# Rose-STL-Lab/spherical-dyffusion

Hardware: AMD Instinct MI355X
Metric: forecast-steps/sec (180x360, 63ch), 25-member ensemble DYffusion sampling, whole job (higher is better)
Workload: dtype f32 tensors; every GEMM-class kernel (1x1 convs, fused MLP, Legendre analysis/synthesis, dhconv) as 3-pass split-f16 MFMA with f32 accumulation; FFT / norms / pointwise in f32 (statistics f64); 1 GPU; 25-member ensemble x horizon-6 DYffusion sampling pass (6 forecaster + 10 interpolator SFNO forwards, dropout stream on, AR feedback), 180x360, 63 state + 2 forcing channels, embed 256, 8 blocks; horizon=6, relayed_members=0, parallelism=members of one initial condition sharded over GPUs, no data-path collective

## Files before the change

### spherical-dyffusion_amd/csrc/mlp_h3.hip

```cpp
#include <cstdlib>
#include <vector>
#include <cmath>
#include <type_traits>

#include "common.h"

typedef const sdy_f16x8 __attribute__((address_space(1)))* wptr_t;
typedef _Float16 f16x4 __attribute__((ext_vector_type(4)));

namespace {

constexpr int ME = 256;
constexpr int MH = 512;
constexpr int TN = 64;
constexpr int HC = 128;
constexpr int NCH = MH / HC;
constexpr int KS1 = ME / 16;
constexpr int KSC = HC / 16;
constexpr int RING = 16;
constexpr int NGROUPS = NCH * 2 * RING;
static_assert(KS1 == RING && 2 * KSC == RING, "ring slot = index inside a block");
constexpr float SX = SDY_ACT_SX;

struct MlpParams {
  const float* x; long x_bs;
  int x_tiled;
  const float* pa; const float* pd;
  const sdy_f16x8* w;
  const float* b1; const float* b2;
  float* out; long out_bs;
  const float* add; long add_bs;
  const float* add_a; const float* add_d;
  int HW, B;
  float s1, s2;
  uint32_t drop_thr; float drop_scale;
  uint32_t seed_lo, seed_hi, stream1, stream2, call, batch_offset;
  int rows_per_call;
  const float* batch_scale;
  double* stats;
  const float* keep_h; const float* keep_o;
  unsigned* flags;
  unsigned* head;
  unsigned long long* stamps;
  SdyImgMap omap;
  int add_local;
};

__device__ __forceinline__ int px_swz(int px) { return (px & 15) ^ (((px >> 4) & 1) * 3); }
__device__ __forceinline__ int xs_off(int px, int c) { return px * ME + (((c & 16) | ((c ^ px_swz(px)) & 15)) << 3); }
__device__ __forceinline__ int hs_off(int px, int c) { return px * HC + (((c ^ px_swz(px)) & 15) << 3); }

template <bool DROP, bool INJECT = false>
__global__ __launch_bounds__(256, 1) void mlp_h3_kernel(const MlpParams p) {
  extern __shared__ __attribute__((aligned(16))) unsigned char smem[];
  _Float16* Xs_hi = reinterpret_cast<_Float16*>(smem);
  _Float16* Xs_lo = Xs_hi + TN * ME;
  _Float16* Hs = Xs_lo + TN * ME;
  float* Cf = reinterpret_cast<float*>(Hs + 4 * TN * HC);
  float* Cb2 = Cf + 4 * ME;

  const int tid = threadIdx.x, lane = tid & 63;
  const int wave = __builtin_amdgcn_readfirstlane(tid >> 6);
  int h = lane >> 5, l31 = lane & 31;
  const int tpi = (p.HW + TN - 1) / TN;
  const int ntiles = tpi * p.B;
  const int t_per = (ntiles + (int)gridDim.x - 1) / (int)gridDim.x;
  const int t_begin = (int)blockIdx.x * t_per;
  const int t_end = (t_begin + t_per < ntiles) ? t_begin + t_per : ntiles;
  int z = 0, zo = 0, n0 = 0;
  bool full = true;

  sdy_f16x8 r_hi[RING], r_lo[RING];
  auto wbase_of = [&](int ln) { return (wptr_t)(p.w + (size_t)wave * (NGROUPS + RING) * SDY_GROUP + ln); };
  wptr_t wp = wbase_of(lane);
#pragma unroll
  for (int s = 0; s < RING; ++s) {
    r_hi[s] = wp[s * SDY_GROUP];
    r_lo[s] = wp[s * SDY_GROUP + 64];
  }
  wp += RING * SDY_GROUP;

  int q0 = tid & 15, o0 = tid >> 4;
  f32x4 xr[2][8];
  const float* pf_base = nullptr;
  const float* res_base = nullptr;
  unsigned pf_off = 0u;
  int pf_rs = 0;
  auto prefetch_setup = [&](int t) {
    const int zz = t / tpi, nn = (t - zz * tpi) * TN;
    const bool ok = nn + 4 * q0 < p.HW;
    pf_base = p.x + (long)zz * p.x_bs + (p.x_tiled ? (long)(t - zz * tpi) * (ME * TN) : 0L);
    pf_rs = p.x_tiled ? TN : p.HW;
    pf_off = p.x_tiled ? (unsigned)(8 * o0 * TN + 4 * q0) * 4u : (unsigned)(8 * o0 * p.HW + (ok ? nn + 4 * q0 : 0)) * 4u;
  };
  auto prefetch_piece = [&](int piece) {
    const int oc = piece >> 3, e = piece & 7;
    xr[oc][e] = sdy_ld16s(pf_base + (long)(8 * 16 * oc + e) * pf_rs, pf_off);
  };
  auto prefetch_x = [&](int t) {
    const int zz = t / tpi, nn = (t - zz * tpi) * TN;
    const bool ok = nn + 4 * q0 < p.HW;
    const float* xz = p.x + (long)zz * p.x_bs + (p.x_tiled ? (long)(t - zz * tpi) * (ME * TN) : 0L);
    const int rs = p.x_tiled ? TN : p.HW;
    const unsigned xo = p.x_tiled ? (unsigned)(8 * o0 * TN + 4 * q0) * 4u : (unsigned)(8 * o0 * p.HW + (ok ? nn + 4 * q0 : 0)) * 4u;
#pragma unroll
    for (int oc = 0; oc < 2; ++oc)
#pragma unroll
      for (int e = 0; e < 8; ++e) xr[oc][e] = sdy_ld16s(xz + (long)(8 * 16 * oc + e) * rs, xo);
  };
  auto load_coeffs = [&](int zz) {
    const int t = 64 * wave + (int)__builtin_amdgcn_mbcnt_hi(~0u, __builtin_amdgcn_mbcnt_lo(~0u, 0u));
    const long c = (long)zz * ME + t, co = (long)sdy_img(p.omap, zz) * ME + t;
    Cf[t] = p.pa ? p.pa[c] * SX : SX;
    Cf[ME + t] = p.pa ? p.pd[c] * SX : 0.0f;
    Cf[2 * ME + t] = p.add_a ? p.add_a[co] : 1.0f;
    Cf[3 * ME + t] = p.add_a ? p.add_d[co] : 0.0f;
  };
  Cb2[tid] = DROP ? p.b2[tid] * p.drop_scale : p.b2[tid];
  if (t_begin < t_end) load_coeffs(t_begin / tpi);
  __syncthreads();
  if (t_begin < t_end) prefetch_x(t_begin);
  double psum[16], psq[16];
#pragma unroll
  for (int i = 0; i < 16; ++i) { psum[i] = 0.0; psq[i] = 0.0; }

  for (int tile = t_begin; tile < t_end; ++tile) {
  asm volatile("" : "+v"(l31), "+v"(h), "+v"(q0), "+v"(o0));
  const int tile_it = tile - t_begin;
  auto stamp = [&](int i) {
#if SDY_STAMPS_ON
    if (p.stamps && blockIdx.x == 3 && tid == 0 && tile_it >= 2 && tile_it < 6)
      p.stamps[(tile_it - 2) * 16 + i] = __builtin_amdgcn_s_memtime();
#else
    (void)i; (void)tile_it;
    if (p.stamps && tid == 0) asm volatile("s_nop 0");
#endif
  };
  stamp(0);
  z = tile / tpi;
  zo = sdy_img(p.omap, z);
  n0 = (tile - z * tpi) * TN;
  full = n0 + TN <= p.HW;

  auto stage_x = [&](auto full_t) {
    constexpr bool kFull = decltype(full_t)::value;
    float amax = 0.0f;
    const bool ok = kFull || (n0 + 4 * q0 < p.HW);
#pragma unroll
    for (int oc = 0; oc < 2; ++oc) {
      float av[8], dv[8];
      {
        const int c0 = 8 * (o0 + 16 * oc);
        const f32x4 a0 = *reinterpret_cast<const f32x4*>(Cf + c0), a1 = *reinterpret_cast<const f32x4*>(Cf + c0 + 4);
        const f32x4 d0 = *reinterpret_cast<const f32x4*>(Cf + ME + c0), d1 = *reinterpret_cast<const f32x4*>(Cf + ME + c0 + 4);
#pragma unroll
        for (int e = 0; e < 4; ++e) { av[e] = a0[e]; av[e + 4] = a1[e]; dv[e] = d0[e]; dv[e + 4] = d1[e]; }
      }
#pragma unroll
      for (int pp = 0; pp < 4; ++pp) {
        const int px = 4 * q0 + pp;
        sdy_f16x8 vh, vl;
        float v[8];
#pragma unroll
        for (int e = 0; e < 8; ++e) v[e] = (kFull || ok) ? fmaf(xr[oc][e][pp], av[e], dv[e]) : 0.0f;
        sdy_split8(v, vh, vl, amax);
        const int off = xs_off(px, o0 + 16 * oc);
        *reinterpret_cast<sdy_f16x8*>(Xs_hi + off) = vh;
        *reinterpret_cast<sdy_f16x8*>(Xs_lo + off) = vl;
      }
    }
    sdy_flag_range(p.flags, amax, p.head);
  };
  if (full) stage_x(std::true_type{});
  else stage_x(std::false_type{});
  __syncthreads();

  f32x16 oacc[2][2];
  f32x4 rres[16];
  const int e_col = n0 + 4 * (tid & 15);
  const bool e_ok = full || e_col < p.HW;
  const unsigned e_ro = (unsigned)((tid >> 4) * p.HW + (e_ok ? e_col : 0)) * 4u;

  constexpr bool do_drop = DROP;
  const int zq = zo / p.rows_per_call, zt = zo - zq * p.rows_per_call;
  const uint32_t call_z = p.call + (uint32_t)zq;
  const uint32_t c1_base = (uint32_t)(((uint64_t)(zt + p.batch_offset) * (uint64_t)(MH >> 2)) & 0xFFFFFFFFu);

  f32x16 acc[2];
  f32x4 bv[4];
  auto load_bias = [&](int hc) {
    const int row0 = HC * hc + 32 * wave + 4 * h;
#pragma unroll
    for (int g4 = 0; g4 < 4; ++g4) bv[g4] = *reinterpret_cast<const f32x4*>(p.b1 + row0 + 8 * g4);
  };
#ifndef SDY_MLP_PINNED
#define SDY_MLP_PINNED 1
#endif
  static_assert(SDY_MLP_PINNED, "the ahead-of-time Philox rounds ride on the pinned fc1 loop");
  uint32_t mw[4][4];
  uint32_t ac0 = 0, ac1 = 0, ac2 = 0, ac3 = 0, ak0 = 0, ak1 = 0;
  constexpr int PR = SDY_PHILOX_ROUNDS;
  constexpr int PSTEP = 96 / (4 * PR);
  static_assert(PSTEP >= 2, "at most one round behind every other MFMA of fc1");
  auto philox_ahead = [&](int hc, int idx) {
    const int g4 = idx / PR, rnd = idx % PR;
    if (rnd == 0) {
      const int row0 = HC * hc + 32 * wave + 4 * h;
      ac0 = (uint32_t)(n0 + l31); ac1 = c1_base + (uint32_t)((row0 + 8 * g4) >> 2); ac2 = p.stream1; ac3 = call_z;
      ak0 = p.seed_lo; ak1 = p.seed_hi;
    }
    const uint64_t p0 = (uint64_t)0xD2511F53u * ac0, p1 = (uint64_t)0xCD9E8D57u * ac2;
    const uint32_t m0 = (uint32_t)(p1 >> 32) ^ ac1 ^ ak0, m2 = (uint32_t)(p0 >> 32) ^ ac3 ^ ak1;
    ac0 = m0; ac1 = (uint32_t)p1; ac2 = m2; ac3 = (uint32_t)p0;
    ak0 += 0x9E3779B9u; ak1 += 0xBB67AE85u;
    if (rnd == PR - 1) { mw[g4][0] = ac0; mw[g4][1] = ac1; mw[g4][2] = ac2; mw[g4][3] = ac3; }
  };
  auto fc1 = [&](int hc_fc1) {
#pragma unroll
    for (int j = 0; j < 2; ++j)
#pragma unroll
      for (int r = 0; r < 16; ++r) acc[j][r] = 0.0f;
    sdy_f16x8 bh[2][2], bl[2][2];
    auto ldb1 = [&](int set, int ks, int part) {
      const int j = part & 1;
      const int off = xs_off(32 * j + l31, 2 * ks + h);
      if (part < 2) bh[set][j] = *reinterpret_cast<const sdy_f16x8*>(Xs_hi + off);
      else bl[set][j] = *reinterpret_cast<const sdy_f16x8*>(Xs_lo + off);
    };
#pragma unroll
    for (int part = 0; part < 4; ++part) ldb1(0, 0, part);
#pragma unroll
    for (int ks = 0; ks < KS1; ++ks) {
      const int c = ks & 1;
      if constexpr (SDY_MLP_PINNED) {
      __builtin_amdgcn_sched_barrier(0);
      const sdy_f16x8 a_lo = r_lo[ks], a_hi = r_hi[ks];
#pragma unroll
      for (int k = 0; k < 6; ++k) {
        const int j = k & 1;
        if (SDY_H3_PASSES == 3 || k >= 4)
          acc[j] = __builtin_amdgcn_mfma_f32_32x32x16_f16(k < 2 ? a_lo : a_hi, (k >= 2 && k < 4) ? bl[c][j] : bh[c][j], acc[j], 0, 0, 0);
        if (k < 4) { if (ks + 1 < KS1) ldb1(c ^ 1, ks + 1, k); }
        else if (k == 4) r_lo[ks] = wp[ks * SDY_GROUP + 64];
        else r_hi[ks] = wp[ks * SDY_GROUP];
        if (DROP && !INJECT && (6 * ks + k) % PSTEP == 0 && (6 * ks + k) / PSTEP < 4 * PR) philox_ahead(hc_fc1, (6 * ks + k) / PSTEP);
        __builtin_amdgcn_sched_barrier(0);
      }
      } else {
      if (ks + 1 < KS1) {
#pragma unroll
        for (int part = 0; part < 4; ++part) ldb1(c ^ 1, ks + 1, part);
      }
#pragma unroll
      for (int j = 0; j < 2; ++j) SDY_CROSS_TERM(acc[j] = __builtin_amdgcn_mfma_f32_32x32x16_f16(r_lo[ks], bh[c][j], acc[j], 0, 0, 0));
#pragma unroll
      for (int j = 0; j < 2; ++j) SDY_CROSS_TERM(acc[j] = __builtin_amdgcn_mfma_f32_32x32x16_f16(r_hi[ks], bl[c][j], acc[j], 0, 0, 0));
#pragma unroll
      for (int j = 0; j < 2; ++j) acc[j] = __builtin_amdgcn_mfma_f32_32x32x16_f16(r_hi[ks], bh[c][j], acc[j], 0, 0, 0);
      r_hi[ks] = wp[ks * SDY_GROUP];
      r_lo[ks] = wp[ks * SDY_GROUP + 64];
#pragma unroll
      for (int k = 0; k < 4; ++k) {
        __builtin_amdgcn_sched_group_barrier(0x008, 1, 0);
        __builtin_amdgcn_sched_group_barrier(0x100, 1, 0);
      }
#pragma unroll
      for (int k = 0; k < 2; ++k) {
        __builtin_amdgcn_sched_group_barrier(0x008, 1, 0);
        __builtin_amdgcn_sched_group_barrier(0x020, 1, 0);
      }
      __builtin_amdgcn_sched_barrier(0);
      }
    }
    wp += RING * SDY_GROUP;
  };
  struct Piece {
    float v[4], t[4], e[4], q[4];
  };
  auto keep_h_at = [&](int row, int px) {
    const int pix = (n0 + px < p.HW) ? n0 + px : p.HW - 1;
    return p.keep_h[((long)zo * MH + row) * p.HW + pix] != 0.0f;
  };
  auto chain_stage = [&](Piece& s, int st, int hc, int j, int g4) {
    const int row0 = HC * hc + 32 * wave + 4 * h;
    const int px = 32 * j + l31;
    switch (st) {
      case 0: {
        const f32x4 b4 = bv[g4];
#pragma unroll
        for (int r = 0; r < 4; r += 2) {
          const sdy_gf2 v2 = sdy_gf2{acc[j][4 * g4 + r], acc[j][4 * g4 + r + 1]} * p.s1 + sdy_gf2{b4[r], b4[r + 1]};
          s.v[r] = v2.x; s.v[r + 1] = v2.y;
        }
        break;
      }
      case 1:
#pragma unroll
        for (int r = 0; r < 4; r += 2) {
          const sdy_gf2 v2 = {s.v[r], s.v[r + 1]};
          const sdy_gf2 t2 = __builtin_elementwise_abs(v2) * (0.3275911f * 0.70710678118654752440f) + 1.0f;
          const sdy_gf2 e2 = v2 * v2;
          s.t[r] = t2.x; s.t[r + 1] = t2.y;
          s.e[r] = e2.x; s.e[r + 1] = e2.y;
        }
        break;
      case 2: {
        s.t[0] = __builtin_amdgcn_rcpf(s.t[0]); s.t[1] = __builtin_amdgcn_rcpf(s.t[1]);
        const sdy_gf2 e2 = sdy_gf2{s.e[0], s.e[1]} * (-0.5f * 1.44269504088896340736f);
        s.e[0] = e2.x; s.e[1] = e2.y;
        break;
      }
      case 3: {
        s.t[2] = __builtin_amdgcn_rcpf(s.t[2]); s.t[3] = __builtin_amdgcn_rcpf(s.t[3]);
        const sdy_gf2 e2 = sdy_gf2{s.e[2], s.e[3]} * (-0.5f * 1.44269504088896340736f);
        s.e[2] = e2.x; s.e[3] = e2.y;
        break;
      }
      case 4: s.e[0] = __builtin_amdgcn_exp2f(s.e[0]); s.e[1] = __builtin_amdgcn_exp2f(s.e[1]); break;
      case 5: s.e[2] = __builtin_amdgcn_exp2f(s.e[2]); s.e[3] = __builtin_amdgcn_exp2f(s.e[3]); break;
      case 6:
#pragma unroll
        for (int r = 0; r < 4; r += 2) {
          const sdy_gf2 t2 = {s.t[r], s.t[r + 1]};
          sdy_gf2 q2 = t2 * (1.061405429f * (0.5f * SX)) + (-1.453152027f * (0.5f * SX));
          q2 = q2 * t2 + (1.421413741f * (0.5f * SX));
          s.q[r] = q2.x; s.q[r + 1] = q2.y;
        }
        break;
      case 7:
#pragma unroll
        for (int r = 0; r < 4; r += 2) {
          const sdy_gf2 t2 = {s.t[r], s.t[r + 1]};
          sdy_gf2 q2 = sdy_gf2{s.q[r], s.q[r + 1]} * t2 + (-0.284496736f * (0.5f * SX));
          q2 = q2 * t2 + (0.254829592f * (0.5f * SX));
          s.q[r] = q2.x; s.q[r + 1] = q2.y;
        }
        break;
      case 8:
#pragma unroll
        for (int r = 0; r < 4; r += 2) {
          const sdy_gf2 q2 = sdy_gf2{s.q[r], s.q[r + 1]} * sdy_gf2{s.t[r], s.t[r + 1]} * sdy_gf2{s.e[r], s.e[r + 1]};
          s.q[r] = q2.x; s.q[r + 1] = q2.y;
        }
        break;
      case 9:
#pragma unroll
        for (int r = 0; r < 4; r += 2) {
          const sdy_gf2 v2 = {s.v[r], s.v[r + 1]};
          const sdy_gf2 o2 = v2 * (0.5f * SX) + __builtin_elementwise_abs(v2) * ((0.5f * SX) - sdy_gf2{s.q[r], s.q[r + 1]});
          s.v[r] = o2.x; s.v[r + 1] = o2.y;
        }
        break;
      case 10: {
        if (do_drop) {
#pragma unroll
          for (int r = 0; r < 4; ++r) {
            bool keep;
            if constexpr (INJECT) keep = keep_h_at(row0 + 8 * g4 + r, px);
            else keep = sdy_keep16(mw[g4][r], j, p.drop_thr);
            s.v[r] = keep ? s.v[r] : 0.0f;
          }
        }
        break;
      }
      default: {
        _Float16* Hh = Hs + (hc & 1) * (2 * TN * HC);
        _Float16* Hl = Hh + TN * HC;
        f16x4 vh, vl;
#pragma unroll
        for (int r = 0; r < 4; r += 2) {
          const sdy_f32x2 x2 = {s.v[r], s.v[r + 1]};
          const sdy_f16x2 h2 = __builtin_convertvector(x2, sdy_f16x2);
          const sdy_f16x2 l2 = __builtin_convertvector(x2 - __builtin_convertvector(h2, sdy_f32x2), sdy_f16x2);
          vh[r] = h2[0]; vh[r + 1] = h2[1];
          vl[r] = l2[0]; vl[r + 1] = l2[1];
        }
        const int off = hs_off(px, 4 * wave + g4) + 4 * h;
        *reinterpret_cast<f16x4*>(Hh + off) = vh;
        *reinterpret_cast<f16x4*>(Hl + off) = vl;
      }
    }
  };
  auto chain_slot = [&](Piece& s, int st, int hc, int j, int g4) {
    const int row0 = HC * hc + 32 * wave + 4 * h;
    const int px = 32 * j + l31;
    constexpr float CT = 0.3275911f * 0.70710678118654752440f, KAP = -0.5f * 1.44269504088896340736f, HS = 0.5f * SX;
    constexpr float A5 = 1.061405429f * HS, A4 = -1.453152027f * HS, A3 = 1.421413741f * HS, A2 = -0.284496736f * HS,
                    A1 = 0.254829592f * HS;
    switch (st) {
      case 0: {
        const f32x4 b4 = bv[g4];
#pragma unroll
        for (int r = 0; r < 4; ++r) s.v[r] = fmaf(acc[j][4 * g4 + r], p.s1, b4[r]);
        break;
      }
      case 1:
#pragma unroll
        for (int r = 0; r < 4; ++r) s.t[r] = fmaf(__builtin_fabsf(s.v[r]), CT, 1.0f);
        s.e[0] = s.v[0] * KAP; s.e[1] = s.v[1] * KAP;
        break;
      case 2:
        s.t[0] = __builtin_amdgcn_rcpf(s.t[0]); s.t[1] = __builtin_amdgcn_rcpf(s.t[1]);
        s.e[2] = s.v[2] * KAP; s.e[3] = s.v[3] * KAP;
        s.e[0] *= s.v[0]; s.e[1] *= s.v[1];
        break;
      case 3:
        s.t[2] = __builtin_amdgcn_rcpf(s.t[2]); s.t[3] = __builtin_amdgcn_rcpf(s.t[3]);
        s.e[2] *= s.v[2]; s.e[3] *= s.v[3];
        s.q[0] = fmaf(s.t[0], A5, A4); s.q[1] = fmaf(s.t[1], A5, A4);
        break;
      case 4:
        s.e[0] = __builtin_amdgcn_exp2f(s.e[0]); s.e[1] = __builtin_amdgcn_exp2f(s.e[1]);
        s.q[2] = fmaf(s.t[2], A5, A4); s.q[3] = fmaf(s.t[3], A5, A4);
        s.q[0] = fmaf(s.q[0], s.t[0], A3); s.q[1] = fmaf(s.q[1], s.t[1], A3);
        break;
      case 5:
        s.e[2] = __builtin_amdgcn_exp2f(s.e[2]); s.e[3] = __builtin_amdgcn_exp2f(s.e[3]);
        s.q[2] = fmaf(s.q[2], s.t[2], A3); s.q[3] = fmaf(s.q[3], s.t[3], A3);
        s.q[0] = fmaf(s.q[0], s.t[0], A2); s.q[1] = fmaf(s.q[1], s.t[1], A2);
        break;
      case 6:
        s.q[2] = fmaf(s.q[2], s.t[2], A2); s.q[3] = fmaf(s.q[3], s.t[3], A2);
#pragma unroll
        for (int r = 0; r < 4; ++r) s.q[r] = fmaf(s.q[r], s.t[r], A1);
        break;
      case 7:
#pragma unroll
        for (int r = 0; r < 4; ++r) s.q[r] *= s.t[r];
        s.q[0] = fmaf(-s.q[0], s.e[0], HS); s.q[1] = fmaf(-s.q[1], s.e[1], HS);
        break;
      case 8:
        s.q[2] = fmaf(-s.q[2], s.e[2], HS); s.q[3] = fmaf(-s.q[3], s.e[3], HS);
#pragma unroll
        for (int r = 0; r < 4; ++r) s.q[r] *= __builtin_fabsf(s.v[r]);
        break;
      case 9:
#pragma unroll
        for (int r = 0; r < 4; ++r) s.v[r] = fmaf(s.v[r], HS, s.q[r]);
        if (do_drop) {
#pragma unroll
          for (int r = 0; r < 4; ++r) {
            bool keep;
            if constexpr (INJECT) keep = keep_h_at(row0 + 8 * g4 + r, px);
            else keep = sdy_keep16(mw[g4][r], j, p.drop_thr);
            s.v[r] = keep ? s.v[r] : 0.0f;
          }
        }
        break;
      case 10: {
#pragma unroll
        for (int r = 0; r < 4; r += 2) {
          const sdy_f16x2 h2 = __builtin_convertvector(sdy_f32x2{s.v[r], s.v[r + 1]}, sdy_f16x2);
          s.e[r >> 1] = __builtin_bit_cast(float, h2);
          s.t[r] = s.v[r] - (float)h2[0]; s.t[r + 1] = s.v[r + 1] - (float)h2[1];
        }
        break;
      }
      default: {
        _Float16* Hh = Hs + (hc & 1) * (2 * TN * HC);
        _Float16* Hl = Hh + TN * HC;
        f16x4 vh, vl;
#pragma unroll
        for (int r = 0; r < 4; r += 2) {
          const sdy_f16x2 h2 = __builtin_bit_cast(sdy_f16x2, s.e[r >> 1]);
          const sdy_f16x2 l2 = __builtin_convertvector(sdy_f32x2{s.t[r], s.t[r + 1]}, sdy_f16x2);
          vh[r] = h2[0]; vh[r + 1] = h2[1];
          vl[r] = l2[0]; vl[r + 1] = l2[1];
        }
        const int off = hs_off(px, 4 * wave + g4) + 4 * h;
        *reinterpret_cast<f16x4*>(Hh + off) = vh;
        *reinterpret_cast<f16x4*>(Hl + off) = vl;
      }
    }
  };
#ifndef SDY_MLP_SCALAR_CHAIN
#define SDY_MLP_SCALAR_CHAIN 1
#endif
  auto chain_piece = [&](int hc, int j, int g4) {
    Piece s;
#pragma unroll
    for (int st = 0; st < 12; ++st) chain_stage(s, st, hc, j, g4);
  };
  auto fc2 = [&](int hc2, auto with_chain) {
    constexpr bool CHAIN = decltype(with_chain)::value;
    const _Float16* Hh = Hs + (hc2 & 1) * (2 * TN * HC);
    const _Float16* Hl = Hh + TN * HC;
    sdy_f16x8 bh[2][2], bl[2][2];
    auto ldb = [&](int set, int t) {
#pragma unroll
      for (int j = 0; j < 2; ++j) {
        const int off = hs_off(32 * j + l31, 2 * t + h);
        bh[set][j] = *reinterpret_cast<const sdy_f16x8*>(Hh + off);
        bl[set][j] = *reinterpret_cast<const sdy_f16x8*>(Hl + off);
      }
    };
    auto ldb1 = [&](int set, int t, int part) {
      const int j = part & 1;
      const int off = hs_off(32 * j + l31, 2 * t + h);
      if (part < 2) bh[set][j] = *reinterpret_cast<const sdy_f16x8*>(Hh + off);
      else bl[set][j] = *reinterpret_cast<const sdy_f16x8*>(Hl + off);
    };
    ldb(0, 0);
#pragma unroll
    for (int t = 0; t < KSC; ++t) {
      const int c = t & 1;
      if (!SDY_MLP_PINNED && t + 1 < KSC) ldb(c ^ 1, t + 1);
      __builtin_amdgcn_sched_barrier(0);
      Piece ps;
#pragma unroll
      for (int mi = 0; mi < 2; ++mi) {
        const int s = 2 * t + mi;
#pragma unroll
        for (int k = 0; k < 6; ++k) {
          const int j = k & 1;
          const sdy_f16x8 a = (k < 2) ? r_lo[s] : r_hi[s];
          const sdy_f16x8 b = (k >= 2 && k < 4) ? bl[c][j] : bh[c][j];
          if (SDY_H3_PASSES == 3 || k >= 4) oacc[mi][j] = __builtin_amdgcn_mfma_f32_32x32x16_f16(a, b, oacc[mi][j], 0, 0, 0);
          if (SDY_MLP_PINNED && mi == 0 && k < 4 && t + 1 < KSC) ldb1(c ^ 1, t + 1, k);
          if (SDY_MLP_PINNED && !CHAIN) __builtin_amdgcn_sched_barrier(0);
          if constexpr (CHAIN) {
            if (SDY_MLP_SCALAR_CHAIN) chain_slot(ps, 6 * mi + k, hc2 + 1, t & 1, t >> 1);
            else chain_stage(ps, 6 * mi + k, hc2 + 1, t & 1, t >> 1);
            __builtin_amdgcn_sched_barrier(0);
          }
        }
        r_hi[s] = wp[s * SDY_GROUP];
        r_lo[s] = wp[s * SDY_GROUP + 64];
        __builtin_amdgcn_sched_barrier(0);
      }
    }
    wp += RING * SDY_GROUP;
  };
  using T_ = std::integral_constant<bool, true>;
  using F_ = std::integral_constant<bool, false>;

  stamp(1);
  load_bias(0);
  fc1(0);
  stamp(2);
#pragma unroll
  for (int pc = 0; pc < 8; ++pc) chain_piece(0, pc & 1, pc >> 1);
  stamp(3);
  __syncthreads();
  stamp(4);
  load_bias(1);
  fc1(1);
  stamp(5);
#pragma unroll
  for (int mi = 0; mi < 2; ++mi)
#pragma unroll
    for (int j = 0; j < 2; ++j)
#pragma unroll
      for (int r = 0; r < 16; ++r) oacc[mi][j][r] = 0.0f;
#pragma unroll 1
  for (int hc = 1; hc < NCH; ++hc) {
    fc2(hc - 1, T_{});
    stamp(4 + 2 * hc);
    __syncthreads();
    if (hc < NCH - 1) {
      load_bias(hc + 1);
      fc1(hc + 1);
    }
    stamp(5 + 2 * hc);
  }
  {
    int ln = lane;
    asm volatile("" : "+v"(ln));
    wp = wbase_of(ln);
  }
  asm volatile("" : "+v"(wp));
  {
    const int nt = tile + 1;
    prefetch_setup(nt < t_end ? nt : tile);
  }
  fc2(NCH - 1, F_{});
  stamp(12);
  {
    res_base = p.add ? p.add + (long)(p.add_local ? z : zo) * p.add_bs : p.x + (long)z * p.x_bs;
  }

  {
    const float bscale = p.batch_scale ? p.batch_scale[zo] : 1.0f;
    const float s2e = do_drop ? p.s2 * p.drop_scale * p.drop_scale : p.s2;
    const uint32_t c1_base2 = (uint32_t)(((uint64_t)(zt + p.batch_offset) * (uint64_t)(ME >> 2)) & 0xFFFFFFFFu);
    float* Os = reinterpret_cast<float*>(smem);
#pragma unroll
    for (int mi = 0; mi < 2; ++mi) {
      const int row0 = 64 * wave + 32 * mi + 4 * h;
      f32x4 bv[4];
#pragma unroll
      for (int g4 = 0; g4 < 4; ++g4) bv[g4] = *reinterpret_cast<const f32x4*>(Cb2 + row0 + 8 * g4);
#pragma unroll
      for (int g4 = 0; g4 < 4; ++g4) {
        uint32_t words[4] = {0xFFFFFFFFu, 0xFFFFFFFFu, 0xFFFFFFFFu, 0xFFFFFFFFu};
        if (do_drop && !INJECT) {
          const philox4 w = philox4x32((uint32_t)(n0 + l31), c1_base2 + (uint32_t)((row0 + 8 * g4) >> 2), p.stream2,
                                          call_z, p.seed_lo, p.seed_hi);
          words[0] = w.x; words[1] = w.y; words[2] = w.z; words[3] = w.w;
        }
#pragma unroll
        for (int j = 0; j < 2; ++j) {
          const int px = 32 * j + l31;
#pragma unroll
          for (int r4 = 0; r4 < 4; r4 += 2) {
            sdy_gf2 o = sdy_gf2{oacc[mi][j][4 * g4 + r4], oacc[mi][j][4 * g4 + r4 + 1]} * s2e +
                        sdy_gf2{bv[g4][r4], bv[g4][r4 + 1]};
            if (do_drop) {
              if constexpr (INJECT) {
                const int pix = (n0 + px < p.HW) ? n0 + px : p.HW - 1;
                const float* km = p.keep_o + ((long)zo * ME + row0 + 8 * g4 + r4) * p.HW + pix;
                o = sdy_gf2{km[0] != 0.0f ? o.x : 0.0f, km[p.HW] != 0.0f ? o.y : 0.0f};
              } else {
                o = sdy_gf2{sdy_keep16(words[r4], j, p.drop_thr) ? o.x : 0.0f,
                            sdy_keep16(words[r4 + 1], j, p.drop_thr) ? o.y : 0.0f};
              }
            }
            o = o * bscale;
            Os[(row0 + 8 * g4 + r4) * TN + px] = o.x;
            Os[(row0 + 8 * g4 + r4 + 1) * TN + px] = o.y;
          }
        }
        {
          const int i0 = 2 * (4 * mi + g4);
          rres[i0] = sdy_ld16s(res_base + (long)(16 * i0) * p.HW, e_ro);
          rres[i0 + 1] = sdy_ld16s(res_base + (long)(16 * (i0 + 1)) * p.HW, e_ro);
          prefetch_piece(i0);
          prefetch_piece(i0 + 1);
        }
      }
    }
    stamp(13);
    __syncthreads();
    stamp(14);
    if (e_ok) {
      float* oz = p.out + (long)zo * p.out_bs;
      const float* os = Os + (tid >> 4) * TN + 4 * (tid & 15);
#pragma unroll
      for (int i = 0; i < 16; ++i) {
        const int row = (tid >> 4) + 16 * i;
        f32x4 v = *reinterpret_cast<const f32x4*>(os + 16 * i * TN);
        if (p.add) v += rres[i] * Cf[2 * ME + row] + Cf[3 * ME + row];
        sdy_st16s(oz + (long)(16 * i) * p.HW, e_ro, v);
        if (p.stats) {
          psum[i] += (double)sdy_quad_sum(v);
          psq[i] += (double)sdy_quad_sumsq(v);
        }
      }
    }
    if (p.stats) {
      const int nt = tile + 1;
      if (nt >= t_end || nt / tpi != z) {
#pragma unroll
        for (int i = 0; i < 16; ++i) {
          double s1 = psum[i], s2 = psq[i];
#pragma unroll
          for (int m = 1; m < 16; m <<= 1) {
            s1 += __shfl_xor(s1, m, 64);
            s2 += __shfl_xor(s2, m, 64);
          }
          if ((tid & 15) == 0) {
            double* st = p.stats + ((long)zo * ME + (tid >> 4) + 16 * i) * 2;
            __hip_atomic_fetch_add(st, s1, __ATOMIC_RELAXED, __HIP_MEMORY_SCOPE_AGENT);
            __hip_atomic_fetch_add(st + 1, s2, __ATOMIC_RELAXED, __HIP_MEMORY_SCOPE_AGENT);
          }
          psum[i] = 0.0; psq[i] = 0.0;
        }
      }
    }
  }
  stamp(15);
  __syncthreads();
  {
    const int nt = tile + 1;
    if (nt < t_end && nt / tpi != z) {
      load_coeffs(nt / tpi);
      __syncthreads();
    }
  }
  }
}

}

#ifndef SDY_MLP_INJECT_TU
#if SDY_STAMPS_ON
static unsigned long long* g_stamps = nullptr;
SDY_DEBUG_EXPORT int sdy_mlp_h3_debug_stamps(unsigned long long* host64) {
  if (!g_stamps || !host64) return SDY_ERR_STATE;
  SDY_HIP_TRY(hipDeviceSynchronize());
  SDY_HIP_TRY(hipMemcpy(host64, g_stamps, 64 * sizeof(unsigned long long), hipMemcpyDeviceToHost));
  return SDY_OK;
}
#endif

extern "C" int sdy_mlp_h3_supported(int E, int hidden) { return (E == ME && hidden == MH) ? 1 : 0; }

extern "C" size_t sdy_mlp_h3_pack_bytes(int E, int hidden) {
  if (!sdy_mlp_h3_supported(E, hidden)) return 0;
  return (size_t)4 * (NGROUPS + RING) * SDY_GROUP * sizeof(sdy_f16x8);
}

extern "C" int sdy_mlp_h3_pack(const float* w1_host, const float* w2_host, int E, int hidden, void* packed_dev,
                               float* scale1, float* scale2) {
  if (!w1_host || !w2_host || !packed_dev || !scale1 || !scale2) return SDY_ERR_ARG;
  if (!sdy_mlp_h3_supported(E, hidden)) return SDY_ERR_UNSUPPORTED;
  const float s1 = sdy_h3_scale(sdy_h3_absmax(w1_host, (size_t)E * hidden));
  const float s2 = sdy_h3_scale(sdy_h3_absmax(w2_host, (size_t)E * hidden));
  const size_t gh = (size_t)SDY_GROUP * 8;
  std::vector<_Float16> buf((size_t)4 * (NGROUPS + RING) * gh, (_Float16)0.0f);
  for (int w = 0; w < 4; ++w) {
    _Float16* d = buf.data() + (size_t)w * (NGROUPS + RING) * gh;
    auto put_fc1 = [&](int hc) {
      for (int ks = 0; ks < KS1; ++ks, d += gh) {
        const float* blk = w1_host + (size_t)(128 * hc + 32 * w) * ME + 16 * ks;
        sdy_h3_put_group(d, s1, [&](int r, int k) { return blk[(size_t)r * ME + k]; });
      }
    };
    auto put_fc2 = [&](int hc) {
      for (int t = 0; t < KSC; ++t)
        for (int mi = 0; mi < 2; ++mi, d += gh) {
          const float* blk = w2_host + (size_t)(64 * w + 32 * mi) * MH + 16 * (KSC * hc + t);
          sdy_h3_put_group(d, s2, [&](int r, int k) { return blk[(size_t)r * MH + k]; });
        }
    };
    put_fc1(0);
    put_fc1(1);
    for (int hc = 1; hc < NCH; ++hc) {
      put_fc2(hc - 1);
      if (hc < NCH - 1) put_fc1(hc + 1);
    }
    put_fc2(NCH - 1);
  }
  SDY_HIP_TRY(hipMemcpy(packed_dev, buf.data(), buf.size() * sizeof(_Float16), hipMemcpyHostToDevice));
  *scale1 = s1;
  *scale2 = s2;
  return SDY_OK;
}

#endif

int sdy_mlp_h3_inject(const sdy_mlp_args* a, void* stream);

#ifdef SDY_MLP_INJECT_TU
int sdy_mlp_h3_inject(const sdy_mlp_args* a, void* stream) {
#else
extern "C" int sdy_mlp_h3(const sdy_mlp_args* a, void* stream) {
  if (a && (a->keep_hidden || a->keep_out)) {
    if (!a->keep_hidden || !a->keep_out || !(a->drop_p > 0.0f)) return SDY_ERR_ARG;
    return sdy_mlp_h3_inject(a, stream);
  }
#endif
  if (!a || !a->x || !a->w || !a->b1 || !a->b2 || !a->out) return SDY_ERR_ARG;
  if (a->B <= 0 || a->HW <= 0) return SDY_ERR_ARG;
  if (!sdy_mlp_h3_supported(a->E, a->hidden)) return SDY_ERR_UNSUPPORTED;
  if ((a->pa == nullptr) != (a->pd == nullptr) || (a->add_a == nullptr) != (a->add_d == nullptr)) return SDY_ERR_ARG;
  if ((a->HW & 3) || (a->x_bstride & 3) || (a->out_bstride & 3) || (a->add && (a->add_bstride & 3))) return SDY_ERR_ALIGN;
  if ((long)a->HW * ME * 4 >= (1L << 32)) return SDY_ERR_UNSUPPORTED;
  if (a->drop_p < 0.0f || a->drop_p >= 1.0f) return SDY_ERR_ARG;
  if (a->B > 65535) return SDY_ERR_UNSUPPORTED;
  MlpParams p{};
  p.x = a->x; p.x_bs = a->x_bstride; p.x_tiled = a->x_tiled; p.pa = a->pa; p.pd = a->pd;
  if (a->x_tiled && !a->add) return SDY_ERR_ARG;
  p.w = reinterpret_cast<const sdy_f16x8*>(a->w);
  p.b1 = a->b1; p.b2 = a->b2;
  p.out = a->out; p.out_bs = a->out_bstride; p.add = a->add; p.add_bs = a->add_bstride;
  p.add_a = a->add ? a->add_a : nullptr; p.add_d = a->add ? a->add_d : nullptr;
  p.HW = a->HW; p.B = a->B;
  p.s1 = 1.0f / (a->w1_scale * SX);
  p.s2 = 1.0f / (a->w2_scale * SX);
  if (a->drop_p > 0.0f) {
    p.drop_thr = sdy_drop_threshold16(a->drop_p);
    if (p.drop_thr == 0u) p.drop_thr = 1u;
    p.drop_scale = 1.0f / (1.0f - a->drop_p);
  }
  p.seed_lo = (uint32_t)(a->seed & 0xFFFFFFFFu); p.seed_hi = (uint32_t)(a->seed >> 32);
  p.stream1 = a->stream_fc1; p.stream2 = a->stream_fc2; p.call = a->call; p.batch_offset = a->batch_offset;
  if (a->rows_per_call < 0 || (!a->out_rows && a->rows_per_call > 0 && a->B % a->rows_per_call)) return SDY_ERR_ARG;
  if (a->out_rows && a->rows_per_call == 0) return SDY_ERR_ARG;
  p.rows_per_call = a->rows_per_call > 0 ? a->rows_per_call : a->B;
  p.batch_scale = a->batch_scale;
  p.stats = a->stats;
  p.keep_h = a->keep_hidden; p.keep_o = a->keep_out;
  if (a->out_rows && !a->add) return SDY_ERR_ARG;
  if (a->add_by_launch_row && (!a->out_rows || a->add_a)) return SDY_ERR_ARG;
  p.add_local = a->add_by_launch_row ? 1 : 0;
  SDY_TRY(sdy_img_map_fill(p.omap, a->out_rows, a->B));
  SDY_TRY(sdy_flags_ptr(&p.flags));
  SDY_TRY(sdy_headroom_ptr(SDY_RANGE_MLP, &p.head));
  p.stamps = nullptr;
#if SDY_STAMPS_ON && !defined(SDY_MLP_INJECT_TU)
  if (std::getenv("SDY_MLP_STAMPS")) {
    if (!g_stamps) SDY_HIP_TRY(hipMalloc(&g_stamps, 64 * sizeof(unsigned long long)));
    p.stamps = g_stamps;
  }
#endif
  int n_cu = 0;
  SDY_TRY(sdy_cu_count(&n_cu));
  const long ntiles = (long)((a->HW + TN - 1) / TN) * a->B;
  dim3 grid((unsigned)(ntiles < n_cu ? ntiles : n_cu));
  constexpr size_t smem = (size_t)(2 * TN * ME + 4 * TN * HC) * sizeof(_Float16) + 5 * ME * sizeof(float);
  static SdyOncePerDevice once;
  std::atomic<bool>* attr_done = nullptr;
  SDY_TRY(once.slot(&attr_done));
#ifdef SDY_MLP_INJECT_TU
  if (!*attr_done) {
    SDY_HIP_TRY(hipFuncSetAttribute(reinterpret_cast<const void*>(&mlp_h3_kernel<true, true>),
                                    hipFuncAttributeMaxDynamicSharedMemorySize, (int)smem));
    *attr_done = true;
  }
  hipLaunchKernelGGL((mlp_h3_kernel<true, true>), grid, dim3(256), smem, (hipStream_t)stream, p);
#else
  if (!*attr_done) {
    SDY_HIP_TRY(hipFuncSetAttribute(reinterpret_cast<const void*>(&mlp_h3_kernel<false>),
                                    hipFuncAttributeMaxDynamicSharedMemorySize, (int)smem));
    SDY_HIP_TRY(hipFuncSetAttribute(reinterpret_cast<const void*>(&mlp_h3_kernel<true>),
                                    hipFuncAttributeMaxDynamicSharedMemorySize, (int)smem));
    *attr_done = true;
  }
  if (p.drop_thr != 0u)
    hipLaunchKernelGGL(mlp_h3_kernel<true>, grid, dim3(256), smem, (hipStream_t)stream, p);
  else
    hipLaunchKernelGGL(mlp_h3_kernel<false>, grid, dim3(256), smem, (hipStream_t)stream, p);
#endif
  return sdy_launch_status();
}
```

Measured before the change: 163.4 member-forecast-steps/s.

## Stage next tile's x split into swapped LDS region during output epilogue

The shared-memory x image and the hidden double buffer now swap regions each tile. This lets the f16 hi/lo split of the next tile's input be written to the free region while the current tile's output rows are stored. The aim is to remove the serial staging phase and its barrier at the top of each tile by overlapping it with epilogue global stores. In exchange, coefficient loading is split into x and add halves, with an extra sync when the image changes, and correctness now depends on careful region aliasing.

Result: no change. 163.6 member-forecast-steps/s, median of 6 (+0.1%).

```diff
diff --git a/spherical-dyffusion_amd/csrc/mlp_h3.hip b/spherical-dyffusion_amd/csrc/mlp_h3.hip
--- a/spherical-dyffusion_amd/csrc/mlp_h3.hip
+++ b/spherical-dyffusion_amd/csrc/mlp_h3.hip
@@ -21,6 +21,20 @@
 constexpr int NGROUPS = NCH * 2 * RING;
 static_assert(KS1 == RING && 2 * KSC == RING, "ring slot = index inside a block");
 constexpr float SX = SDY_ACT_SX;
+constexpr unsigned REGION = 2 * TN * ME * sizeof(_Float16);
+static_assert(REGION == 4 * TN * HC * sizeof(_Float16), "the x image and the hidden double buffer exchange storage");
+#ifdef SDY_MLP_NO_REGION_SWAP
+constexpr bool SWAP = false;
+#else
+constexpr bool SWAP = true;
+#endif
+#ifndef SDY_MLP_SPLIT0_AT
+#define SDY_MLP_SPLIT0_AT 16
+#endif
+#ifndef SDY_MLP_SPLIT1_AT
+#define SDY_MLP_SPLIT1_AT 16
+#endif
+static_assert(0 <= SDY_MLP_SPLIT0_AT && SDY_MLP_SPLIT0_AT <= SDY_MLP_SPLIT1_AT && SDY_MLP_SPLIT1_AT <= 16, "store rounds");
 
 struct MlpParams {
   const float* x; long x_bs;
@@ -53,10 +67,8 @@
 template <bool DROP, bool INJECT = false>
 __global__ __launch_bounds__(256, 1) void mlp_h3_kernel(const MlpParams p) {
   extern __shared__ __attribute__((aligned(16))) unsigned char smem[];
-  _Float16* Xs_hi = reinterpret_cast<_Float16*>(smem);
-  _Float16* Xs_lo = Xs_hi + TN * ME;
-  _Float16* Hs = Xs_lo + TN * ME;
-  float* Cf = reinterpret_cast<float*>(Hs + 4 * TN * HC);
+  unsigned xreg = 0u;
+  float* Cf = reinterpret_cast<float*>(smem + 2 * REGION);
   float* Cb2 = Cf + 4 * ME;
 
   const int tid = threadIdx.x, lane = tid & 63;
@@ -108,21 +120,68 @@
 #pragma unroll
       for (int e = 0; e < 8; ++e) xr[oc][e] = sdy_ld16s(xz + (long)(8 * 16 * oc + e) * rs, xo);
   };
-  auto load_coeffs = [&](int zz) {
+  auto load_coeffs = [&](int zz, bool x_half, bool add_half) {
     const int t = 64 * wave + (int)__builtin_amdgcn_mbcnt_hi(~0u, __builtin_amdgcn_mbcnt_lo(~0u, 0u));
     const long c = (long)zz * ME + t, co = (long)sdy_img(p.omap, zz) * ME + t;
-    Cf[t] = p.pa ? p.pa[c] * SX : SX;
-    Cf[ME + t] = p.pa ? p.pd[c] * SX : 0.0f;
-    Cf[2 * ME + t] = p.add_a ? p.add_a[co] : 1.0f;
-    Cf[3 * ME + t] = p.add_a ? p.add_d[co] : 0.0f;
+    if (x_half) {
+      Cf[t] = p.pa ? p.pa[c] * SX : SX;
+      Cf[ME + t] = p.pa ? p.pd[c] * SX : 0.0f;
+    }
+    if (add_half) {
+      Cf[2 * ME + t] = p.add_a ? p.add_a[co] : 1.0f;
+      Cf[3 * ME + t] = p.add_a ? p.add_d[co] : 0.0f;
+    }
+  };
+  auto stage_half = [&](auto full_t, int oc, _Float16* Xh, _Float16* Xl, int nn, float& amax) {
+    constexpr bool kFull = decltype(full_t)::value;
+    const bool ok = kFull || (nn + 4 * q0 < p.HW);
+    float av[8], dv[8];
+    {
+      const int c0 = 8 * (o0 + 16 * oc);
+      const f32x4 a0 = *reinterpret_cast<const f32x4*>(Cf + c0), a1 = *reinterpret_cast<const f32x4*>(Cf + c0 + 4);
+      const f32x4 d0 = *reinterpret_cast<const f32x4*>(Cf + ME + c0), d1 = *reinterpret_cast<const f32x4*>(Cf + ME + c0 + 4);
+#pragma unroll
+      for (int e = 0; e < 4; ++e) { av[e] = a0[e]; av[e + 4] = a1[e]; dv[e] = d0[e]; dv[e + 4] = d1[e]; }
+    }
+#pragma unroll
+    for (int pp = 0; pp < 4; ++pp) {
+      const int px = 4 * q0 + pp;
+      sdy_f16x8 vh, vl;
+      float v[8];
+#pragma unroll
+      for (int e = 0; e < 8; ++e) v[e] = (kFull || ok) ? fmaf(xr[oc][e][pp], av[e], dv[e]) : 0.0f;
+      sdy_split8(v, vh, vl, amax);
+      const int off = xs_off(px, o0 + 16 * oc);
+      *reinterpret_cast<sdy_f16x8*>(Xh + off) = vh;
+      *reinterpret_cast<sdy_f16x8*>(Xl + off) = vl;
+    }
+  };
+  auto stage_x = [&](bool full_tile, _Float16* Xh, _Float16* Xl, int nn) {
+    float amax = 0.0f;
+    if (full_tile) {
+      stage_half(std::true_type{}, 0, Xh, Xl, nn, amax);
+      stage_half(std::true_type{}, 1, Xh, Xl, nn, amax);
+    } else {
+      stage_half(std::false_type{}, 0, Xh, Xl, nn, amax);
+      stage_half(std::false_type{}, 1, Xh, Xl, nn, amax);
+    }
+    sdy_flag_range(p.flags, amax, p.head);
   };
   Cb2[tid] = DROP ? p.b2[tid] * p.drop_scale : p.b2[tid];
-  if (t_begin < t_end) load_coeffs(t_begin / tpi);
+  if (t_begin < t_end) load_coeffs(t_begin / tpi, true, true);
   __syncthreads();
   if (t_begin < t_end) prefetch_x(t_begin);
   double psum[16], psq[16];
 #pragma unroll
   for (int i = 0; i < 16; ++i) { psum[i] = 0.0; psq[i] = 0.0; }
+  if (SWAP) {
+    if (t_begin < t_end) {
+      const int nn = (t_begin - (t_begin / tpi) * tpi) * TN;
+      _Float16* Xh = reinterpret_cast<_Float16*>(smem);
+      stage_x(false, Xh, Xh + TN * ME, nn);
+    }
+    __syncthreads();
+  }
 
   for (int tile = t_begin; tile < t_end; ++tile) {
   asm volatile("" : "+v"(l31), "+v"(h), "+v"(q0), "+v"(o0));
@@ -142,38 +201,13 @@
   n0 = (tile - z * tpi) * TN;
   full = n0 + TN <= p.HW;
 
-  auto stage_x = [&](auto full_t) {
-    constexpr bool kFull = decltype(full_t)::value;
-    float amax = 0.0f;
-    const bool ok = kFull || (n0 + 4 * q0 < p.HW);
-#pragma unroll
-    for (int oc = 0; oc < 2; ++oc) {
-      float av[8], dv[8];
-      {
-        const int c0 = 8 * (o0 + 16 * oc);
-        const f32x4 a0 = *reinterpret_cast<const f32x4*>(Cf + c0), a1 = *reinterpret_cast<const f32x4*>(Cf + c0 + 4);
-        const f32x4 d0 = *reinterpret_cast<const f32x4*>(Cf + ME + c0), d1 = *reinterpret_cast<const f32x4*>(Cf + ME + c0 + 4);
-#pragma unroll
-        for (int e = 0; e < 4; ++e) { av[e] = a0[e]; av[e + 4] = a1[e]; dv[e] = d0[e]; dv[e + 4] = d1[e]; }
-      }
-#pragma unroll
-      for (int pp = 0; pp < 4; ++pp) {
-        const int px = 4 * q0 + pp;
-        sdy_f16x8 vh, vl;
-        float v[8];
-#pragma unroll
-        for (int e = 0; e < 8; ++e) v[e] = (kFull || ok) ? fmaf(xr[oc][e][pp], av[e], dv[e]) : 0.0f;
-        sdy_split8(v, vh, vl, amax);
-        const int off = xs_off(px, o0 + 16 * oc);
-        *reinterpret_cast<sdy_f16x8*>(Xs_hi + off) = vh;
-        *reinterpret_cast<sdy_f16x8*>(Xs_lo + off) = vl;
-      }
-    }
-    sdy_flag_range(p.flags, amax, p.head);
-  };
-  if (full) stage_x(std::true_type{});
-  else stage_x(std::false_type{});
-  __syncthreads();
+  _Float16* Xs_hi = reinterpret_cast<_Float16*>(smem + xreg);
+  _Float16* Xs_lo = Xs_hi + TN * ME;
+  _Float16* Hs = reinterpret_cast<_Float16*>(smem + (SWAP ? xreg ^ REGION : REGION));
+  if (!SWAP) {
+    stage_x(full, Xs_hi, Xs_lo, n0);
+    __syncthreads();
+  }
 
   f32x16 oacc[2][2];
   f32x4 rres[16];
@@ -583,7 +617,7 @@
     const float bscale = p.batch_scale ? p.batch_scale[zo] : 1.0f;
     const float s2e = do_drop ? p.s2 * p.drop_scale * p.drop_scale : p.s2;
     const uint32_t c1_base2 = (uint32_t)(((uint64_t)(zt + p.batch_offset) * (uint64_t)(ME >> 2)) & 0xFFFFFFFFu);
-    float* Os = reinterpret_cast<float*>(smem);
+    float* Os = reinterpret_cast<float*>(Xs_hi);
 #pragma unroll
     for (int mi = 0; mi < 2; ++mi) {
       const int row0 = 64 * wave + 32 * mi + 4 * h;
@@ -632,21 +666,45 @@
     stamp(13);
     __syncthreads();
     stamp(14);
-    if (e_ok) {
-      float* oz = p.out + (long)zo * p.out_bs;
-      const float* os = Os + (tid >> 4) * TN + 4 * (tid & 15);
-#pragma unroll
-      for (int i = 0; i < 16; ++i) {
-        const int row = (tid >> 4) + 16 * i;
-        f32x4 v = *reinterpret_cast<const f32x4*>(os + 16 * i * TN);
-        if (p.add) v += rres[i] * Cf[2 * ME + row] + Cf[3 * ME + row];
-        sdy_st16s(oz + (long)(16 * i) * p.HW, e_ro, v);
-        if (p.stats) {
-          psum[i] += (double)sdy_quad_sum(v);
-          psq[i] += (double)sdy_quad_sumsq(v);
-        }
-      }
-    }
+    const int nt_s = tile + 1;
+    const bool split_next = SWAP && nt_s < t_end;
+    const int zn = nt_s / tpi, nn = (nt_s - zn * tpi) * TN;
+    const bool full_n = nn + TN <= p.HW;
+    if (split_next && zn != z) {
+      load_coeffs(zn, true, false);
+      __syncthreads();
+    }
+    _Float16* Xn_hi = reinterpret_cast<_Float16*>(smem + (xreg ^ REGION));
+    _Float16* Xn_lo = Xn_hi + TN * ME;
+    float amax_n = 0.0f;
+    auto split_half = [&](int oc) {
+      if (split_next) {
+        if (full_n) stage_half(std::true_type{}, oc, Xn_hi, Xn_lo, nn, amax_n);
+        else stage_half(std::false_type{}, oc, Xn_hi, Xn_lo, nn, amax_n);
+      }
+    };
+    constexpr int S0 = SWAP ? SDY_MLP_SPLIT0_AT : 16, S1 = SWAP ? SDY_MLP_SPLIT1_AT : 16;
+#pragma unroll
+    for (int seg = 0; seg < 3; ++seg) {
+      const int i_begin = seg == 0 ? 0 : seg == 1 ? S0 : S1, i_end = seg == 0 ? S0 : seg == 1 ? S1 : 16;
+      if (i_begin < i_end && e_ok) {
+        float* oz = p.out + (long)zo * p.out_bs;
+        const float* os = Os + (tid >> 4) * TN + 4 * (tid & 15);
+#pragma unroll
+        for (int i = i_begin; i < i_end; ++i) {
+          const int row = (tid >> 4) + 16 * i;
+          f32x4 v = *reinterpret_cast<const f32x4*>(os + 16 * i * TN);
+          if (p.add) v += rres[i] * Cf[2 * ME + row] + Cf[3 * ME + row];
+          sdy_st16s(oz + (long)(16 * i) * p.HW, e_ro, v);
+          if (p.stats) {
+            psum[i] += (double)sdy_quad_sum(v);
+            psq[i] += (double)sdy_quad_sumsq(v);
+          }
+        }
+      }
+      if (SWAP && seg < 2) split_half(seg);
+    }
+    if (split_next) sdy_flag_range(p.flags, amax_n, p.head);
     if (p.stats) {
       const int nt = tile + 1;
       if (nt >= t_end || nt / tpi != z) {
@@ -673,10 +731,11 @@
   {
     const int nt = tile + 1;
     if (nt < t_end && nt / tpi != z) {
-      load_coeffs(nt / tpi);
-      __syncthreads();
-    }
-  }
+      load_coeffs(nt / tpi, !SWAP, true);
+      if (!SWAP) __syncthreads();
+    }
+  }
+  if (SWAP) xreg ^= REGION;
   }
 }
 
```
